# sanazkaviani/3d-latent-diffusion-model

Measured on AMD Instinct MI355X. Metric: UNet denoising steps/sec (bf16, 1x4x24x24x24 latent; whole job = sum over GPUs), higher is better.
Workload: dtype bf16

## Files before the change

### 3d-latent-diffusion-model_amd/csrc/ldm3d.hip

```cpp
#include <hip/hip_runtime.h>
#include <dlfcn.h>
#include <math.h>
#include <stdarg.h>
#include <stdio.h>
#include <stdlib.h>
#include <string.h>

#include <algorithm>
#include <atomic>
#include <map>
#include <memory>
#include <string>
#include <type_traits>
#include <vector>

#include "../../include/ldm3d.h"
#include "attention.h"
#include "conv_igemm.h"
#include "conv_halo.h"
#include "conv_cube.h"
#ifdef LDM_EXPERIMENTS
#include "conv_halo_pp.h"
#include "conv_halo_rw.h"
#endif
#include "conv_thin.h"
#include "gemm_light.h"
#include "gemm_light_x3.h"
#include "conv_block.h"
#include "conv_wgrad.h"
#include "conv_wgrad_w16.h"
#include "conv_wgrad_kw3.h"
#include "norm_elem.h"
#include "window.h"
#include "metrics.h"
#include "fin_gn.h"
#include "f32_path.h"
#include "f32_train.h"

#ifndef CONV_STAGES
#define CONV_STAGES 4
#endif

static thread_local char g_err[1024] = "";
static int fail(int code, const char* fmt, ...) {
    va_list ap; va_start(ap, fmt); vsnprintf(g_err, sizeof g_err, fmt, ap); va_end(ap);
    return code;
}
#define HIP_TRY(x) do { hipError_t e_ = (x); if (e_ != hipSuccess) \
    return fail(LDM_ERR_HIP, "%s failed: %s (%s:%d)", #x, hipGetErrorString(e_), __FILE__, __LINE__); } while (0)
#define LDM_TRY(x) do { int r_ = (x); if (r_ != 0) return r_; } while (0)


#ifdef LDM_EXPERIMENTS
// ... 68 lines not shown
struct Ref { int base = BASE_NULL; size_t off = 0; };
static inline Ref ws_ref(size_t off) { Ref r; r.base = BASE_WS; r.off = off; return r; }
static inline Ref w_ref(size_t off) { Ref r; r.base = BASE_W; r.off = off; return r; }
static inline Ref io_ref(int i) { Ref r; r.base = BASE_IO0 + i; r.off = 0; return r; }
static inline Ref w32_ref(size_t off) { Ref r; r.base = BASE_W32; r.off = 2 * off; return r; }

struct Act {
    size_t off = 0; int C = 0; int N = 0, D = 0, H = 0, W = 0; bool valid = false;
    size_t stats_off = 0; bool has_stats = false;
    int stats_nrb = 0;
    int esz = 2;
    bool hl = false;
    size_t cs_off = 0; int cs_rows = 0;
    size_t bytes() const { return (size_t)N * D * H * W * C * esz; }
    long rows() const { return (long)N * D * H * W; }
};

enum OpKind { OP_PACK, OP_CONV, OP_FINALIZE, OP_GN_STATS, OP_GN_FINALIZE, OP_GN_PREP, OP_GN_APPLY, OP_ATTN, OP_SINUSOID,
              OP_GEMV, OP_VAE_HEADS, OP_GN_FUSED,
              OP_WT , OP_WT_BATCH, OP_WGRAD, OP_EXPORT , OP_EXPORT_BATCH, OP_COLSUM, OP_GNB, OP_ATTN_BWD, OP_ADD, OP_SUMPOOL, OP_LIN_DX, OP_LIN_DW, OP_VAE_HEADS_BWD,
              OP_GEMM_LIGHT,
              OP_COLSUM_BATCH,
              OP_IM2COL,
              OP_PACK32, OP_CONV32, OP_FIN32, OP_GN_STATS32, OP_GN_APPLY32, OP_ATTN32, OP_GEMV32,
              OP_TAP,
              OP_BUCKET, OP_BUCKET_JOIN,
              OP_UPS_SPLIT32,
              OP_CONV_THIN,
              OP_FIN_GN,
              OP_GEMM_LIGHT32,
              OP_CONV_BLOCK,
              OP_TEMB_ROW };

struct ConvCfg { int wgm, wgn, bk, splitk; int halo = 0, mtps = 0, qps = 0; int slab_lg = 0; int cube = 0; int th = 0, big = 0; };

struct ConvRec {
    Ref xa, xb, w; int ca, cb;
    Ref x1a, x1b, w1; int c1a, c1b;
    int N, Din, Hin, Win, Dout, Hout, Wout;
    int k, stride, pad, M;
    int couts, cout_pad, cout_real;
    int nchunk0, nchunk1, mtiles, ntiles;
    bool ups, exact;
    bool phase;
    bool x3;
    bool ep32_ndhwc, ep32_ncdhw;
    Ref bias, bias2, temb, residual; int temb_stride;
    Ref out; int f32_out;
    Ref partial, stats;
    int stats_nrb, stats_rows;
    Ref gamma, beta, gn_out; int gn_groups, gn_silu, gn_lg; float gn_eps;
};

struct GnRec {
    Ref xa, xb; int ca, cb, N, DHW;
    Ref gamma, beta; int groups; float eps; bool silu;
    Ref stats_a, stats_b; int nrb_a, nrb_b;
    Ref partial; int nslab, rows_per_slab;
    Ref ab, mr;
    Ref out; bool out_hl;
    int rows_per_block, chunks;
    Ref dy, gsum, dgamma_n, dbeta_n;
    Ref cs; bool leaves_colsums;
    Ref acc_a, acc_b, dxa, dxb;
    int dgamma_flat, dbeta_flat;
    bool fp32;
    int count, out_stride; bool over_n;
// ... 278 lines not shown
        const ConvW* w = nullptr;
        int k = 3, stride = 1, pad = 1, ups = 0;
        int Do = 0, Ho = 0, Wo = 0;
        Act g1a, g1b; const ConvW* w1 = nullptr;
        Ref temb; int temb_stride = 0;
        Act residual;
        bool f32_out = false; Ref out_ref; int cout_real = 0;
        bool want_stats = true;
        Ref w_over; bool no_bias = false; int exact = 0;
        int temb_row = -1;
        int f32_tag = 0;
    };
    struct Tape {
        int kind = 0;
        ConvArgs c; Act out; bool leaf_input = false;
        const GnW* g = nullptr; Act xa, xb; size_t ab_off = 0, mr_off = 0; int groups = 0; bool silu = false;
        Act qkv, o; size_t lse_off = 0; int head_ch = 64;
    };
    std::vector<Tape> tape;

    static bool halo_enabled() { return ldm_knob("LDM_CONV_HALO", 1) != 0; }
    static int tall_mode() { return ldm_xknob("LDM_HALO_TALL", 2); }
    static bool light_enabled() { return ldm_knob("LDM_GEMM_LIGHT", 1) != 0; }
    static bool two_wg_enabled() { return ldm_knob("LDM_IGEMM_2WG", 1) != 0; }
    static bool phase_enabled() { return ldm_knob("LDM_CONV_PHASE", 1) != 0; }
    static bool halo_skip_enabled() { static const int v = ldm_knob("LDM_HALO_SKIP", 1); return v != 0; }
    static bool halo_skip_split_enabled() { static const int v = ldm_knob("LDM_HALO_SKIP_SPLIT", 1); return v != 0; }
    static bool cube_enabled() { return ldm_knob("LDM_CONV_CUBE", 1) != 0; }
    static bool cube_ok(int D, int H, int W, int cin0, int c1a, int c1b, int cout_pad) {
        return cube_enabled() && D >= 1 && H >= 1 && W >= 1 && D <= CUBE_EDGE && H <= CUBE_EDGE && W <= CUBE_EDGE && cin0 % 64 == 0 && cin0 >= 128 &&
               c1a % 64 == 0 && c1b % 64 == 0 && cout_pad % 16 == 0;
    }
    static ConvCfg cube_cfg(int cin0) { ConvCfg c{2, 2, 64, cin0 / 64}; c.cube = 1; return c; }
    static ConvCfg choose_cfg(long M, int cout_pad, int steps0, int bk, int halo_n = 0, long halo_dhw = 0, bool halo_only = false, int steps1 = 0) {
        ConvCfg best{2, 2, bk, 1}; double best_t = 1e30;
        const int steps = steps0 + steps1;
        const int rb = bk * 2;
        static const int splits[] = {1, 2, 3, 4, 6, 8, 9, 12, 16, 18, 24, 27, 32, 48, 64};
        for (int wgn = 1; wgn <= 4 && !halo_only; wgn *= 2) {
            const int bn = 64 * wgn, bm = 64 * (4 / wgn);
            if (cout_pad % bn) continue;
            const long tiles = ((M + bm - 1) / bm) * (cout_pad / bn);
            const double c_mfma = (double)bm * bn * bk * 2.0 / 4096.0;
            const double c_load = (double)(bm + bn) * rb / 28.0;
            const double c_step = std::max(c_mfma, c_load) + 60.0;
            for (int sk : splits) {
                if (sk > 1 && steps / sk < 6) break;
                const long nwg = tiles * sk;
                const int sps = (steps + sk - 1) / sk;
                const double rounds = ceil((double)nwg / 256.0);
                double t = rounds * (sps * c_step + 2500.0);
                if (sk > 1) t += 6000.0 + (double)M * cout_pad * 4.0 * sk * 2.0 / 2500.0;
                if (t < best_t) { best_t = t; best = ConvCfg{4 / wgn, wgn, bk, sk}; }
            }
        }
        if (halo_n > 0 && bk == 64 && cout_pad % 128 == 0 && halo_enabled()) {
            const int mtps = (int)((halo_dhw + 125) / 126), Q = steps0 / 3;
            const long tiles = (long)halo_n * mtps * (cout_pad / 128);
            const double c_mfma = 128.0 * 128.0 * 64.0 * 2.0 / 4096.0;
            const double c_load = (128.0 / 3.0 + 128.0) * 128.0 / 28.0;
            const double c_step = std::max(c_mfma, c_load) + 30.0;
            for (int sk : splits) {
                if (sk > 1 && Q / sk < 3) break;
                const int qps = (Q + sk - 1) / sk, skr = (Q + qps - 1) / qps;
                const long nwg = tiles * skr;
                const double rounds = ceil((double)nwg / 256.0);
// ... 252 lines not shown
                return Act();
            }
        }
        const bool phase = a.ups == 1 && !a.exact && a.k == 3 && a.stride == 1 && a.pad == 1 && !train && !a.xb.valid && !a.w1 &&
                           a.w_over.base == BASE_NULL && w.wp_off != 0 && phase_enabled() &&
                           a.Do == 2 * a.xa.D && a.Ho == 2 * a.xa.H && a.Wo == 2 * a.xa.W;
        if (gemm_light_ok(a.k, a.stride, a.ups, cin0, !a.w1, !a.f32_out && a.temb.base == BASE_NULL) && light_enabled() &&
            a.xa.D == a.Do && a.xa.H == a.Ho && a.xa.W == a.Wo && M * (long)cin0 * 2 < (1L << 31))
            return emit_light(OP_GEMM_LIGHT, a, M, a.w_over.base != BASE_NULL ? a.w_over : w_ref(w.w_off), gemm_light_big(M, w.cout_pad), a.want_stats);
        if (conv_block_enabled() && a.k == 3 && a.stride == 1 && a.pad == 1 && a.ups == 0 && !a.exact && !a.xb.valid && !a.w1 && !a.f32_out &&
            w.cout_pad == 64 && rup(w.cout, 32) == 64 && cin0 <= conv_block_max_cin() &&
            a.xa.D == a.Do && a.xa.H == a.Ho && a.xa.W == a.Wo) {
            const int TH = conv_block_th();
            const int td = (a.Do + BLK_TD - 1) / BLK_TD, th = (a.Ho + TH - 1) / TH, tw = (a.Wo + BLK_TW - 1) / BLK_TW;
            static const long min_blocks = ldm_knob("LDM_CONV_BLOCK_MIN", 512L);
            if ((long)N * td * th * tw >= min_blocks) return emit_conv_block(a, M, TH, td * th * tw);
        }
        if (conv_block128_enabled() && a.k == 3 && a.stride == 1 && a.pad == 1 && a.ups == 0 && !a.exact && !a.xb.valid && !a.w1 && !a.f32_out &&
            w.cout_pad == 128 && rup(w.cout, 32) == 128 && cin0 <= conv_block128_max_cin() && a.xa.D == a.Do && a.xa.H == a.Ho && a.xa.W == a.Wo) {
            const int td = (a.Do + BLK_TD - 1) / BLK_TD, th = (a.Ho + 7) / 8, tw = (a.Wo + BLK_TW - 1) / BLK_TW;
            static const long min_blocks = ldm_knob("LDM_CONV_BLOCK128_MIN", 192L);
            static const long max_blocks = ldm_xknob("LDM_CONV_BLOCK128_MAX", 0L);
            const long tiles128 = (long)N * td * th * tw;
            if (tiles128 >= min_blocks && tiles128 <= (max_blocks > 0 ? max_blocks : (long)device_cus())) return emit_conv_block(a, M, 8, td * th * tw);
        }
        const int taps = phase ? 8 : a.k * a.k * a.k;
        const bool halo_ok = a.k == 3 && a.stride == 1 && a.pad == 1 && a.ups == 0 && !a.exact && !a.xb.valid && (!a.w1 || (halo_skip_enabled() && bk == 64)) &&
                             a.xa.D == a.Do && a.xa.H == a.Ho && a.xa.W == a.Wo;
        int nchunk0 = cin0 / bk, nchunk1 = cin1 / bk;
        int steps0 = taps * nchunk0, steps1 = nchunk1;
        ConvCfg cc = choose_cfg(M, w.cout_pad, steps0, bk, halo_ok ? N : 0, (long)a.Do * a.Ho * a.Wo, false, steps1);
        if (halo_ok && bk == 64 && !hp && !train && !phase && cube_ok(a.Do, a.Ho, a.Wo, cin0, a.w1 ? a.g1a.C : 0, (a.w1 && a.g1b.valid) ? a.g1b.C : 0, w.cout_pad))
            cc = cube_cfg(cin0);
        const int bm = 64 * cc.wgm, bn = 64 * cc.wgn;
        const int couts = a.f32_out ? 0 : rup(w.cout, 32);
        const int mtiles_pp = (int)(((long)a.xa.D * a.xa.H * a.xa.W + bm - 1) / bm);
        if (!cc.halo && cc.bk == 64 && cc.wgm <= 2 && cc.splitk == 1 && two_wg_enabled() && steps0 + steps1 <= 64 &&
            (phase ? (long)N * 8 * mtiles_pp : (M + bm - 1) / bm) * (w.cout_pad / bn) >= 512) {
            cc.bk = 32; nchunk0 = cin0 / 32; nchunk1 = cin1 / 32; steps0 = taps * nchunk0; steps1 = nchunk1;
        }
        Act out;
        if (!a.f32_out) {
            out = new_act(N, a.Do, a.Ho, a.Wo, couts);
            if (a.want_stats) {
                const long dhwo = (long)a.Do * a.Ho * a.Wo;
                if (cc.splitk > 1) {
                    out.stats_off = pool.alloc((size_t)((M + 31) / 32) * couts * 2 * 4); out.has_stats = true; out.stats_nrb = 0;
                } else if (cc.halo) {
                    out.stats_off = pool.alloc((size_t)N * cc.mtps * couts * 2 * 4); out.has_stats = true; out.stats_nrb = cc.mtps;
                } else if (phase) {
                    out.stats_off = pool.alloc((size_t)N * 8 * mtiles_pp * couts * 2 * 4); out.has_stats = true; out.stats_nrb = 8 * mtiles_pp;
                } else if (N == 1 || dhwo % bm == 0) {
                    out.stats_off = pool.alloc((size_t)((M + bm - 1) / bm) * couts * 2 * 4); out.has_stats = true;
                    out.stats_nrb = (int)(N == 1 ? (M + bm - 1) / bm : dhwo / bm);
                }
            }
        }
        Op op{}; op.kind = OP_CONV; op.cc = cc;
        ConvRec& c = op.cv; c = conv_rec(a, phase ? 2 : a.k, a.stride, a.pad, M, a.cout_real ? a.cout_real : w.cout);
        conv_epilogue(c, a, out); conv_sources(c, a);
        c.w = a.w_over.base != BASE_NULL ? a.w_over : w_ref(phase ? w.wp_off : w.w_off);
        if (a.w1) {
            c.x1a = ws_ref(a.g1a.off); c.c1a = a.g1a.C; c.w1 = w_ref(a.w1->w_off); c.bias2 = w_ref(a.w1->b_off);
            if (a.g1b.valid) { c.x1b = ws_ref(a.g1b.off); c.c1b = a.g1b.C; }
        }
        c.stats = out.has_stats ? ws_ref(out.stats_off) : Ref();
        c.phase = phase; c.ups = !phase && (a.ups & 1); c.exact = !phase && (a.exact & 1);
        c.nchunk0 = nchunk0; c.nchunk1 = nchunk1;
        c.mtiles = cc.halo ? N * cc.mtps : phase ? N * 8 * mtiles_pp : (int)((M + bm - 1) / bm);
        if (M >= (1L << 31)) { err = "conv " + tag + ": M too large"; return Act(); }
        if (cc.splitk > 1) { partial_bytes = std::max(partial_bytes, (size_t)cc.splitk * M * w.cout_pad * 4); partial_fixups.push_back(plan->ops.size()); }
        plan->ops.push_back(op);
        if (cc.splitk > 1) { Op f = op; f.kind = OP_FINALIZE; partial_fixups.push_back(plan->ops.size()); plan->ops.push_back(f); }
        record_conv(a, out);
        return out;
    }

    static bool fin_gn_enabled() { static const int v = ldm_knob("LDM_FIN_GN", 1); return v != 0; }
    std::map<size_t, Act> prenorm;
    bool fuse_fin_gn(Act& raw, bool keep_raw, const GnW& g, int groups, float eps, bool silu, Act* y) {
// ... 1089 lines not shown
#define ABL_CASE(A) if ((p.dbg & 508) == A) { \
            HIP_TRY(hipFuncSetAttribute(reinterpret_cast<const void*>(&conv3_halo_kernel<6, A>), hipFuncAttributeMaxDynamicSharedMemorySize, LDS)); \
            hipLaunchKernelGGL((conv3_halo_kernel<6, A>), dim3(p.mtiles * p.ntiles * p.splitk), dim3(512), LDS, s, p); return 0; }
        if ((p.dbg & 508) == 384) {
            constexpr int LDSX = LDS + 64;
            if (p.dbg & 2048) {
                HIP_TRY(hipFuncSetAttribute(reinterpret_cast<const void*>(&conv3_halo_kernel<6, 385>), hipFuncAttributeMaxDynamicSharedMemorySize, LDSX));
                hipLaunchKernelGGL((conv3_halo_kernel<6, 385>), dim3(p.mtiles * p.ntiles * p.splitk), dim3(512), LDSX, s, p); return 0;
            }
            HIP_TRY(hipFuncSetAttribute(reinterpret_cast<const void*>(&conv3_halo_kernel<6, 384>), hipFuncAttributeMaxDynamicSharedMemorySize, LDSX));
            hipLaunchKernelGGL((conv3_halo_kernel<6, 384>), dim3(p.mtiles * p.ntiles * p.splitk), dim3(512), LDSX, s, p); return 0;
        }
        ABL_CASE(4) ABL_CASE(8) ABL_CASE(16) ABL_CASE(12) ABL_CASE(20) ABL_CASE(24) ABL_CASE(32) ABL_CASE(40) ABL_CASE(84) ABL_CASE(68) ABL_CASE(64) ABL_CASE(128) ABL_CASE(256)
#undef ABL_CASE
    }
    if (loop) hipLaunchKernelGGL((conv3_halo_kernel<6, 0, false, true>), dim3(grid), dim3(512), LDS, s, p);
    else if (mi) hipLaunchKernelGGL((conv3_halo_kernel<6, 0, false, false, true>), dim3(grid), dim3(512), LDS, s, p);
    else hipLaunchKernelGGL((conv3_halo_kernel<6>), dim3(grid), dim3(512), LDS, s, p);
    return 0;
}

static int launch_conv_cube(const ConvParams& p, hipStream_t s) {
    if (p.c0a % 64 || p.x0b || p.x3_n || p.splitk != p.c0a / 64 || p.splitk < 2 || p.CoutPad % 16 || p.Dout > CUBE_EDGE || p.Hout > CUBE_EDGE ||
        p.Wout > CUBE_EDGE || p.c1a % 64 || p.c1b % 64 || !p.partial)
        return fail(LDM_ERR_BAD_ARG, "conv3_cube_kernel: unsupported conv (cin %d, splitk %d, %dx%dx%d)", p.c0a, p.splitk, p.Dout, p.Hout, p.Wout);
    static bool attr_tab[32] = {}; bool& attr_set = attr_flag(attr_tab);
    if (!attr_set) {
        HIP_TRY(hipFuncSetAttribute(reinterpret_cast<const void*>(&conv3_cube_kernel), hipFuncAttributeMaxDynamicSharedMemorySize, CUBE_LDS));
        attr_set = true;
    }
    hipLaunchKernelGGL(conv3_cube_kernel, dim3(p.splitk, p.CoutPad / 16, p.N), dim3(256), CUBE_LDS, s, p);
    return 0;
}
static int launch_conv_impl(const ConvParams& p, const ConvCfg& cc, hipStream_t s) {
    if (cc.cube) return launch_conv_cube(p, s);
    if (cc.halo) return launch_conv_halo(p, s, cc.halo == 2);
#define CASE(M_, N_, K_) if (cc.wgm == M_ && cc.wgn == N_ && cc.bk == K_) return launch_conv_t<M_, N_, K_>(p, s);
    CASE(2, 2, 64) CASE(4, 1, 64) CASE(1, 4, 64) CASE(2, 2, 32) CASE(4, 1, 32) CASE(1, 4, 32)
#undef CASE
    return fail(LDM_ERR_BAD_ARG, "no conv kernel for tile config %dx%d bk %d", cc.wgm, cc.wgn, cc.bk);
}

static inline int grid_for(long total, int per_block = 256, int cap = 4096) {
    long g = (total + per_block - 1) / per_block; if (g > cap) g = cap; if (g < 1) g = 1; return (int)g;
}

static void conv32_cfg(long M, int cout_pad, int steps, bool x3, int* bn_out, int* sk_out) {
    static const int f32_bn = ldm_knob("LDM_F32_BN", 0);
    static const int f32_wgs = ldm_knob("LDM_F32_WGS", 512);
    const int mtiles = (int)((M + 127) / 128);
    int bn = (cout_pad % 128) ? 64 : 128;
    if (f32_bn == 64 || (f32_bn == 1 && (long)mtiles * (cout_pad / 128) < 256)) bn = 64;
    const long tiles = (long)mtiles * ((cout_pad + bn - 1) / bn);
    int sk = 1;
    if (tiles < f32_wgs * 3 / 4) {
        sk = (int)std::min<long>(std::max<long>(1, f32_wgs / tiles), std::max(1, steps / (x3 ? 4 : 8)));
        const int sps = (steps + sk - 1) / sk; sk = (steps + sps - 1) / sps;
    }
    *bn_out = bn; *sk_out = sk;
}
static int fin32_stats_blocks(int N, int dhwo, int couts, int* rows) {
    const int cvec = couts / 4, rows_par = std::max(1, 256 / cvec);
    int nrb = std::min((dhwo + rows_par - 1) / rows_par, std::max(1, 256 / N));
    *rows = (dhwo + nrb - 1) / nrb;
    return (dhwo + *rows - 1) / *rows;
}
static void launch_conv32(const Conv32Params& p, bool x3, int bn, hipStream_t s) {
    const dim3 grid(p.mtiles * p.ntiles * p.splitk);
// ... 199 lines not shown
template <class P> static P wgrad_params(const WgradRec& w, const Bases& bs) {
    P p{}; p.dy = (decltype(p.dy))rp(bs, w.dy); p.cdy = w.cdy; p.x = (decltype(p.x))rp(bs, w.x); p.cx = w.cx;
    p.dw = (float*)rp(bs, w.dw); p.Cout = w.Cout; p.Cin = w.Cin; p.dw_ld = w.dw_ld; p.dw_ci_off = w.dw_ci_off;
    p.N = w.N; p.Din = w.Din; p.Hin = w.Hin; p.Win = w.Win; p.Dout = w.Dout; p.Hout = w.Hout; p.Wout = w.Wout;
    p.ksize = w.ksize; p.stride = w.stride; p.pad = w.pad; p.ups = w.ups; p.M = w.M;
    p.co_tiles = (p.Cout + 127) / 128; p.ci_tiles = (p.Cin + 127) / 128; p.ksplit = w.ksplit;
    p.slab_stride = (long)w.ksize * w.ksize * w.ksize * w.rows_total * w.dw_ld;
    return p;
}

struct PlanTrace { bool on = false; std::string path; PlanTrace() { const char* e = getenv("LDM_PLAN_TRACE"); if (e && *e) { on = true; path = e; } } };
static PlanTrace g_plan_trace;
struct LaneCtx { GradSyncState* sync = nullptr; };

static int run_plan(const Plan& plan, const Bases& bs, const int* rt, hipStream_t s, size_t begin = 0, size_t end = (size_t)-1,
                    LaneCtx lanes = LaneCtx()) {
    if (end > plan.ops.size()) end = plan.ops.size();
    const char* trace_path = g_plan_trace.on ? g_plan_trace.path.c_str() : nullptr;
    std::vector<hipEvent_t> tev;
    if (trace_path) { tev.resize(end - begin + 1); for (auto& e : tev) HIP_TRY(hipEventCreate(&e)); }
    struct TraceDone {
        const Plan& plan; size_t begin, end; std::vector<hipEvent_t>& ev; hipStream_t s; const char* path;
        ~TraceDone() {
            if (ev.empty()) return;
            (void)hipEventRecord(ev.back(), s); (void)hipEventSynchronize(ev.back());
            FILE* f = fopen(path, "a");
            for (size_t oi = begin; oi < end && f; ++oi) {
                const Op& o = plan.ops[oi]; float ms = 0.f; (void)hipEventElapsedTime(&ms, ev[oi - begin], ev[oi - begin + 1]);
                fprintf(f, "%zu,%zu,%d,%.3f", plan.ops.size(), oi, (int)o.kind, ms * 1e3f);
                const ConvRec& c = o.cv;
                if (o.kind == OP_CONV || o.kind == OP_FINALIZE)
                    fprintf(f, ",M=%d k=%d s=%d ups=%d cin=%d+%d(x%d) cin1=%d couts=%d cfg=%dx%dx%d splitk=%d halo=%d mtps=%d qps=%d cube=%d", c.M, c.k, c.stride,
                            c.ups | c.exact << 1 | c.phase << 2 | c.x3 << 3 | c.ep32_ndhwc << 4 | c.ep32_ncdhw << 5, c.ca, c.cb, c.nchunk0, c.c1a + c.c1b, c.couts,
                            o.cc.wgm, o.cc.wgn, o.cc.bk, o.cc.splitk, o.cc.halo, o.cc.mtps, o.cc.qps, o.cc.cube);
                else {
                    const GnRec& g = o.gn; const WgradRec& w = o.wg;
                    int v[6] = {o.i[0], o.i[1], o.i[2], o.i[3], o.i[4], o.i[5]};
                    auto six = [&](int a, int b, int c2, int d, int e, int h) { v[0] = a; v[1] = b; v[2] = c2; v[3] = d; v[4] = e; v[5] = h; };
                    switch (o.kind) {
                        case OP_FIN_GN: six(c.gn_groups, c.gn_silu, c.gn_lg, c.c1b, c.N, c.Din); break;
                        case OP_CONV32: case OP_FIN32: six(c.ca, c.cb, c.stats_nrb, c.stats_rows, c.N, c.Din); break;
                        case OP_CONV_THIN: six(c.N, c.Din, c.Hin, c.Win, c.x3 ? c.ca / 2 * 3 : c.ca, c.cout_pad); break;
                        case OP_CONV_BLOCK: six(c.N, c.Dout, c.Hout, c.Wout, c.ca, o.cc.th); break;
                        case OP_GEMM_LIGHT: case OP_GEMM_LIGHT32: six(c.M, c.ca + c.cb, c.couts, c.cout_pad, o.cc.big, c.ca); break;
                        case OP_GN_STATS: case OP_GN_STATS32: six(g.ca, g.cb, g.DHW, g.nslab, g.rows_per_slab, g.N); break;
                        case OP_GN_FINALIZE: six(g.nslab, g.ca + g.cb, g.groups, g.DHW, g.N, 0); break;
                        case OP_GN_PREP: six(g.ca, g.cb, g.nrb_a, g.groups, g.DHW, g.N); break;
                        case OP_GN_FUSED: six(g.ca, g.cb, g.nrb_a, g.nrb_b, g.groups, g.DHW); break;
                        case OP_GN_APPLY: six(g.ca, g.cb, g.DHW, g.N, g.silu, 0); break;
                        case OP_GN_APPLY32: six(g.ca, g.cb, g.DHW, g.N, g.silu, g.nrb_a ? 1 : g.nslab); break;
                        case OP_COLSUM: six(g.N, g.nslab, g.ca, g.over_n, g.count, g.out_stride); break;
                        case OP_GNB: six(g.ca, g.cb, g.groups, g.DHW, g.N, g.silu); break;
                        case OP_WGRAD: six(w.cdy, w.cx, w.Cout, w.Cin, w.dw_ld, w.dw_ci_off); break;
                        default: break;
                    }
                    fprintf(f, ",i=%d %d %d %d %d %d", v[0], v[1], v[2], v[3], v[4], v[5]);
                }
                fprintf(f, "\n");
            }
            if (f) fclose(f);
            for (auto e : ev) (void)hipEventDestroy(e);
        }
    } trace_done{plan, begin, end, tev, s, trace_path};
    for (size_t oi = begin; oi < end; ++oi) {
        const Op& o = plan.ops[oi];
        const int* i = o.i;
        if (trace_path) HIP_TRY(hipEventRecord(tev[oi - begin], s));
// ... 1338 lines not shown
    for (auto& e : g_prof.ev) HIP_TRY(hipEventCreate(&e));
    g_prof.wgm = wgm; g_prof.wgn = wgn; g_prof.bk = bk & 0xff; g_prof.halo = (bk >> 8) & 1; g_prof.on = true;
    return 0;
}
int ldm_profile_detail(double* flops, double* ms, int max) {
    if (!flops || !ms || max < 0) return fail(LDM_ERR_BAD_ARG, "null argument");
    const int n = (int)(g_prof.used / 2);
    for (int k = 0; k < n && k < max; ++k) {
        HIP_TRY(hipEventSynchronize(g_prof.ev[2 * k + 1]));
        float t = 0.f; HIP_TRY(hipEventElapsedTime(&t, g_prof.ev[2 * k], g_prof.ev[2 * k + 1]));
        flops[k] = g_prof.flops[k]; ms[k] = t;
    }
    return n;
}
int ldm_profile_stop(double out[5]) {
    if (!out) return fail(LDM_ERR_BAD_ARG, "null out");
    g_prof.on = false;
    double ms = 0.0, fl = 0.0;
    for (size_t k = 0; k + 1 < g_prof.used + 1 && k < g_prof.used; k += 2) {
        HIP_TRY(hipEventSynchronize(g_prof.ev[k + 1]));
        float t = 0.f; HIP_TRY(hipEventElapsedTime(&t, g_prof.ev[k], g_prof.ev[k + 1]));
        ms += t; fl += g_prof.flops[k / 2];
    }
    out[0] = (double)(g_prof.used / 2); out[1] = ms; out[2] = fl; out[3] = (double)g_prof.launches_all; out[4] = g_prof.flops_all;
    for (auto e : g_prof.ev) (void)hipEventDestroy(e);
    g_prof.ev.clear(); g_prof.used = 0; g_prof.flops.clear();
    return 0;
}
int ldm_model_plan_conv_cfgs(ldm_model* m, const char* kind, int B, int D, int H, int W, int* cfgs, int max_convs) {
    if (!m || !kind) return fail(LDM_ERR_BAD_ARG, "null argument");
    std::shared_ptr<Plan> p; LDM_TRY(get_plan(m, kind, B, D, H, W, &p));
    int n = 0;
    for (const Op& o : p->ops) if (o.kind == OP_CONV) {
        if (cfgs && n < max_convs) { cfgs[4 * n] = o.cc.wgm; cfgs[4 * n + 1] = o.cc.wgn; cfgs[4 * n + 2] = o.cc.bk | ((o.cc.cube ? 5 : o.cc.halo) << 8); cfgs[4 * n + 3] = o.cc.splitk; }
        ++n;
    } else if (o.kind == OP_CONV_BLOCK) {
        if (cfgs && n < max_convs) { cfgs[4 * n] = 4; cfgs[4 * n + 1] = o.cv.couts == 128 ? 2 : 1; cfgs[4 * n + 2] = 32 | ((o.cv.couts == 128 ? 4 : 3) << 8); cfgs[4 * n + 3] = 1; }
        ++n;
    }
    return n;
}

int ldm_model_plan_launches(ldm_model* m, const char* kind, int B, int D, int H, int W) {
    if (!m || !kind) return fail(LDM_ERR_BAD_ARG, "null argument");
    std::shared_ptr<Plan> p; LDM_TRY(get_plan(m, kind, B, D, H, W, &p));
    int n = 0;
    for (const Op& o : p->ops) if (o.kind != OP_TAP) ++n;
    return n;
}

static char* g_zero_page = nullptr;
static int ensure_zero_page() {
    if (g_zero_page) return 0;
    HIP_TRY(hipMalloc((void**)&g_zero_page, 8192));
    HIP_TRY(hipMemset(g_zero_page, 0, 8192));
    HIP_TRY(hipDeviceSynchronize());
    return 0;
}

int ldm_op_conv3d_block128(const void* x, int cin, const void* w, const float* bias, const float* temb, int temb_stride, const void* residual,
                           void* out, float* stats, int N, int D, int H, int W, void* stream) {
    if (!x || !w || !out || N < 1 || D < 1 || H < 1 || W < 1 || cin < 32 || cin % 32) return fail(LDM_ERR_BAD_ARG, "bad argument");
    if ((long)N * D * H * W * cin * 2 >= (1L << 32)) return fail(LDM_ERR_BAD_ARG, "the input tensor exceeds 4 GiB (split the batch)");
    BlockParams q{}; q.x = (const bf16_t*)x; q.w = (const bf16_t*)w; q.bias = bias; q.temb = temb; q.temb_stride = temb_stride;
    q.residual = (const bf16_t*)residual; q.out = (bf16_t*)out; q.stats = stats; q.N = N; q.D = D; q.H = H; q.W = W; q.Cin = cin;
    HIP_TRY(launch_conv_block128(q, (hipStream_t)stream));
    return 0;
// ... 43 lines not shown
    const int Du = Din << ups, Hu = Hin << ups, Wu = Win << ups;
    const int pad_total = (stride == 2 && pad == 0 && ksize == 3) ? 1 : 2 * pad;
    const int Do = (Du + pad_total - ksize) / stride + 1, Ho = (Hu + pad_total - ksize) / stride + 1,
              Wo = (Wu + pad_total - ksize) / stride + 1;
    const long M = (long)N * Do * Ho * Wo;
    if (M >= (1L << 31) || M < 1) return fail(LDM_ERR_BAD_ARG, "bad output size");
    if (!stats && !wgn && !splitk && out_bf16 && !out_f32 && gemm_light_ok(ksize, stride, ups, cin0, cin1 == 0, !temb && !bias2) &&
        Builder::light_enabled() && M * (long)cin0 * 2 < (1L << 31)) {
        LightParams lp{}; lp.x = (const bf16_t*)xa; lp.w = (const bf16_t*)w; lp.bias = bias; lp.residual = (const bf16_t*)residual;
        lp.out = (bf16_t*)out_bf16; lp.stats = nullptr; lp.M = (int)M; lp.K = cin0; lp.CoutS = rup(cout, 32);
        lp.xb = (const bf16_t*)xb; lp.ca = ca;
        HIP_TRY(launch_gemm_light(lp, cout_pad, gemm_light_big(M, cout_pad), (hipStream_t)stream));
        return 0;
    }
    const int taps = ksize * ksize * ksize;
    ConvParams p{};
    p.x0a = (const bf16_t*)xa; p.x0b = (const bf16_t*)xb; p.c0a = ca; p.c0b = cb; p.w0 = (const bf16_t*)w;
    p.x1a = (const bf16_t*)x1a; p.x1b = (const bf16_t*)x1b; p.c1a = c1a; p.c1b = c1b; p.w1 = (const bf16_t*)w1;
    p.zero_page = (const bf16_t*)g_zero_page;
    p.N = N; p.Din = Din; p.Hin = Hin; p.Win = Win; p.Dout = Do; p.Hout = Ho; p.Wout = Wo;
    p.ksize = ksize; p.stride = stride; p.pad = pad; p.ups = ups; p.exact = exact; p.M = (int)M;
    p.CoutS = rup(cout, 32); p.CoutPad = cout_pad; p.CoutReal = cout;
    p.nchunk0 = cin0 / bk; p.nchunk1 = cin1 / bk; p.steps0 = taps * p.nchunk0; p.steps1 = p.nchunk1;
    const bool halo_ok = ksize == 3 && stride == 1 && pad == 1 && ups == 0 && !exact && cb == 0 && bk == 64 &&
                         (cin1 == 0 || (Builder::halo_skip_enabled() && (splitk <= 1 || Builder::halo_skip_split_enabled()))) && Builder::halo_enabled();
    ConvCfg cc = Builder::choose_cfg(M, cout_pad, p.steps0, bk, halo_ok ? N : 0, (long)Do * Ho * Wo, false, p.steps1);
    if (wgn) {
        if ((wgn != 1 && wgn != 2 && wgn != 4) || cout_pad % (64 * wgn)) return fail(LDM_ERR_BAD_ARG, "bad wgn");
        cc.wgn = wgn; cc.wgm = 4 / wgn; cc.halo = (wgn == 2 && halo_ok && cout_pad % 128 == 0) ? 1 : (wgn == 1 && halo_ok && Builder::tall_mode() != 0) ? 2 : 0;
    }
    if (splitk) cc.splitk = splitk;
    if (!wgn && !splitk && halo_ok && !out_f32 && !(ldm_xknob("LDM_CONV_DBG", 0)) && Builder::cube_ok(Do, Ho, Wo, cin0, c1a, c1b, cout_pad))
        cc = Builder::cube_cfg(cin0);
    if (cc.splitk < 1 || cc.splitk > p.steps0 + p.steps1) return fail(LDM_ERR_BAD_ARG, "bad splitk");
    if (cc.halo && !cc.cube) {
        const int Q = 9 * p.nchunk0;
        if (cc.splitk > Q) cc.splitk = Q;
        cc.qps = (Q + cc.splitk - 1) / cc.splitk; cc.splitk = (Q + cc.qps - 1) / cc.qps;
        cc.mtps = (int)(((long)Do * Ho * Wo + (cc.halo == 2 ? 253 : 125)) / (cc.halo == 2 ? 254 : 126));
    }
    p.splitk = cc.splitk; p.steps_per_split = cc.halo ? 3 * cc.qps : (p.steps0 + p.steps1 + cc.splitk - 1) / cc.splitk;
    p.halo_mtps = cc.mtps; p.q_per_split = cc.qps;
    p.mtiles = cc.halo ? N * cc.mtps : (int)((M + 64 * cc.wgm - 1) / (64 * cc.wgm)); p.ntiles = cout_pad / (64 * cc.wgn);
    p.bias = bias; p.bias2 = bias2; p.temb = temb; p.temb_stride = temb_stride; p.residual = (const bf16_t*)residual;
    p.out = out_f32 ? nullptr : (bf16_t*)out_bf16; p.out_f32 = out_f32;
    if (cc.splitk > 1) {
        const size_t need = (size_t)cc.splitk * M * cout_pad * 4;
        if (!scratch || scratch_bytes < need) return fail(LDM_ERR_WORKSPACE, "split-K scratch too small: need %zu bytes", need);
        p.partial = (float*)scratch;
    }
    if (stats) {
        const long dhwo = (long)Do * Ho * Wo; const int bm = 64 * cc.wgm;
        if (out_f32 || !stats_nrb) return fail(LDM_ERR_BAD_ARG, "statistics need the bf16 output form");
        if (cc.splitk > 1) { if (N > 1 && dhwo % 32) return fail(LDM_ERR_UNSUPPORTED, "statistics: DHW %% 32 != 0 with a batch"); *stats_nrb = (int)(N == 1 ? (M + 31) / 32 : dhwo / 32); }
        else if (cc.halo) *stats_nrb = cc.mtps;
        else { if (N > 1 && dhwo % bm) return fail(LDM_ERR_UNSUPPORTED, "statistics: tiles straddle samples"); *stats_nrb = (int)(N == 1 ? (M + bm - 1) / bm : dhwo / bm); }
        p.stats = stats;
    }
    p.dbg = (int)ldm_xknob("LDM_CONV_DBG", 0);
    if (p.dbg & 512) {
        if (cc.splitk > 1 || !scratch || scratch_bytes < (size_t)p.mtiles * p.ntiles * (64 + 4096)) return fail(LDM_ERR_BAD_ARG, "stamps need scratch and splitk 1");
        p.stamps = (unsigned long long*)scratch;
    }
    if (fg && cc.splitk > 1) p.slab_lg = fg->lg;
    LDM_TRY(launch_conv(p, cc, (hipStream_t)stream));
    if (cc.splitk > 1) {
        const FinalizeParams f = finalize_params(p);
        if (fg) {
            fg->f = f; fg->f.stats = nullptr;
            HIP_TRY(launch_fin_gn(*fg, N, wt_stores(), (hipStream_t)stream));
        } else
            launch_finalize(f, stats && wt_stores(), (hipStream_t)stream);
    } else if (fg) return fail(LDM_ERR_UNSUPPORTED, "the fused finalize + GroupNorm needs a conv that is split over K");
    HIP_TRY(hipGetLastError());
    return 0;
}

int ldm_op_conv3d(const void* xa, int ca, const void* xb, int cb, const void* w, const float* bias,
                  const void* x1a, int c1a, const void* x1b, int c1b, const void* w1, const float* bias2,
                  const float* temb, int temb_stride, const void* residual, void* out_bf16, float* out_f32,
                  int N, int Din, int Hin, int Win, int ksize, int stride, int pad, int ups,
                  int cout, int cout_pad, int wgn, int splitk, void* scratch, size_t scratch_bytes, void* stream) {
    return op_conv3d_impl(xa, ca, xb, cb, w, bias, x1a, c1a, x1b, c1b, w1, bias2, temb, temb_stride, residual, out_bf16, out_f32, N, Din, Hin, Win,
                          ksize, stride, pad, ups, cout, cout_pad, wgn, splitk, scratch, scratch_bytes, stream, nullptr, nullptr);
}

size_t ldm_op_conv3d_gn_scratch_bytes(int N, int D, int H, int W, int cout_pad, int splitk) {
// ... 1009 lines not shown
```

Measured before the change: 508.1.

## Add plane-per-workgroup 3x3x3 conv kernel for 12^3 feature maps

Adds a new conv kernel that gives each workgroup one output depth plane and a 16-channel output slice. It stages the three input planes plus all 27 tap weights in LDS through buffer-load-to-LDS with dedicated loader waves, and double-buffers the stages. It covers volumes up to 12^3 that are too large for the cube kernel, and fuses the skip-connection 1x1 conv, bias, temb, residual and per-plane GroupNorm stats. The aim is to replace split-K or halo paths and their finalize passes at mid resolution, at the cost of one-workgroup-per-CU occupancy and a large LDS footprint.

```diff
diff --git a/3d-latent-diffusion-model_amd/csrc/conv_plane.h b/3d-latent-diffusion-model_amd/csrc/conv_plane.h
--- /dev/null
+++ b/3d-latent-diffusion-model_amd/csrc/conv_plane.h
@@ -0,0 +1,230 @@
+#pragma once
+#include <type_traits>
+#include "conv_cube.h"
+
+constexpr int PLANE_EDGE = 12;
+constexpr int PLANE_ROWS = 576;
+constexpr int PLANE_TILES = 10;
+constexpr int PLANE_IMG = PLANE_ROWS * 64;
+constexpr int PLANE_STAGE = PLANE_IMG + 27 * 1024;
+constexpr int PLANE_SROWS = 192;
+constexpr int PLANE_SUNIT = 8 * PLANE_SROWS * 16;
+constexpr int PLANE_SWOFF = 2 * PLANE_SUNIT;
+constexpr int PLANE_RED = 16384;
+constexpr int PLANE_LDS = 2 * PLANE_STAGE;
+static_assert(PLANE_LDS <= 160 * 1024, "LDS budget");
+static_assert(PLANE_ROWS % 64 == 0 && PLANE_SROWS % 64 == 0, "whole LDS-DMA copies; chunk strides a multiple of 16 rows");
+static_assert(PLANE_TILES * 16 >= PLANE_EDGE * (PLANE_EDGE + 1), "tiles cover the domain");
+static_assert(PLANE_TILES * 16 - 1 + 2 * (PLANE_EDGE + 1) * (PLANE_EDGE + 1) + 2 * (PLANE_EDGE + 1) + 2 < PLANE_ROWS, "largest row read");
+static_assert(PLANE_TILES * 16 <= PLANE_SROWS && PLANE_SWOFF + 2 * 2048 <= PLANE_STAGE, "skip stage fits a stage buffer");
+static_assert(PLANE_TILES * 1024 <= PLANE_RED && PLANE_RED + 256 <= PLANE_LDS, "end-of-kernel areas");
+
+__global__ __launch_bounds__(512, 1) __attribute__((amdgpu_waves_per_eu(2, 2))) void conv3_plane_kernel(const ConvParams p) {
+#if defined(__HIP_DEVICE_COMPILE__)
+    extern __shared__ __attribute__((aligned(16))) char smem[];
+    typedef __attribute__((address_space(3))) void* lds_ptr_t;
+    constexpr unsigned OOB = 0x80000000u;
+    const int tid = threadIdx.x, lane = tid & 63;
+    const int wave8 = __builtin_amdgcn_readfirstlane(tid >> 6);
+    const bool loader = wave8 >= 4;
+    const int wave = wave8 & 3;
+    const int n0 = blockIdx.x * 16, d = blockIdx.y, smp = blockIdx.z;
+    if (n0 >= p.CoutS) return;
+    const int D = p.Dout, H = p.Hout, W = p.Wout, DHW = D * H * W, RP = W + 1, PP = (H + 1) * RP, dom = H * RP;
+    const unsigned cin2 = (unsigned)p.c0a * 2u;
+    const int nst0 = p.c0a >> 5, units = p.steps1, nst = nst0 + ((units + 1) >> 1);
+
+    const bf16_t* xs = p.x0a + (size_t)smp * DHW * p.c0a;
+    __amdgpu_buffer_rsrc_t rs_x = __builtin_amdgcn_make_buffer_rsrc((void*)xs, 0, (int)((unsigned)DHW * cin2), 0x00020000);
+    __amdgpu_buffer_rsrc_t rs_w = __builtin_amdgcn_make_buffer_rsrc((void*)p.w0, 0, (int)(27u * (unsigned)p.CoutPad * cin2), 0x00020000);
+    unsigned vo[PLANE_ROWS / 64];
+#pragma unroll
+    for (int i = 0; i < PLANE_ROWS / 64; ++i) {
+        const int r = (wave + 4 * i) * 16 + (lane >> 2);
+        const int pl = r / PP, rem = r - pl * PP, hp = rem / RP, wp = rem - hp * RP, dd = d - 1 + pl;
+        const bool real = pl <= 2 && dd >= 0 && dd < D && hp >= 1 && wp >= 1;
+        vo[i] = real ? (unsigned)((dd * H + hp - 1) * W + wp - 1) * cin2 + (unsigned)(lane & 3) * 16u : OOB;
+    }
+    const unsigned wv = (unsigned)(wave * p.CoutPad + n0 + (lane >> 2)) * cin2 + (unsigned)((lane & 3) ^ ((lane >> 3) & 2)) * 16u;
+    const unsigned wstep = 4u * (unsigned)p.CoutPad * cin2;
+    auto issue_main = [&](const int s, const int b) {
+        char* buf = smem + b * PLANE_STAGE;
+        const unsigned so = (unsigned)s * 64u;
+#pragma unroll
+        for (int i = 0; i < 7; ++i) {
+            const int tap = wave + 4 * i;
+            if (tap < 27) __builtin_amdgcn_raw_ptr_buffer_load_lds(rs_w, (lds_ptr_t)(buf + PLANE_IMG + tap * 1024), 16, wv + (unsigned)i * wstep + so, 0, 0, 0);
+        }
+#pragma unroll
+        for (int i = 0; i < PLANE_ROWS / 64; ++i)
+            __builtin_amdgcn_raw_ptr_buffer_load_lds(rs_x, (lds_ptr_t)(buf + (wave + 4 * i) * 1024), 16, vo[i] + so, 0, 0, 0);
+    };
+    unsigned s_vox[PLANE_SROWS / 64];
+#pragma unroll
+    for (int g = 0; g < PLANE_SROWS / 64; ++g) {
+        const int q = g * 64 + lane;
+        s_vox[g] = OOB;
+        if (q < dom) {
+            const int h = q / RP, w = q - h * RP;
+            if (w < W) s_vox[g] = (unsigned)((d * H + h) * W + w);
+        }
+    }
+    const int nca = p.c1a / 64;
+    const unsigned w1row2 = (unsigned)(p.c1a + p.c1b) * 2u;
+    auto issue_skip = [&](const int j, const int b) {
+        char* buf = smem + b * PLANE_STAGE;
+#pragma unroll
+        for (int ul = 0; ul < 2; ++ul) {
+            const int u = 2 * j + ul;
+            if (u >= units) break;
+            const bool a = u < nca;
+            const bf16_t* src = (a ? p.x1a : p.x1b) + (size_t)smp * DHW * (a ? p.c1a : p.c1b);
+            const unsigned row2 = (unsigned)(a ? p.c1a : p.c1b) * 2u, jc = (unsigned)(a ? u : u - nca) * 128u;
+            __amdgpu_buffer_rsrc_t rs_s = __builtin_amdgcn_make_buffer_rsrc((void*)src, 0, (int)((unsigned)DHW * row2), 0x00020000);
+#pragma unroll
+            for (int i = 0; i < 2 * (PLANE_SROWS / 64); ++i) {
+                const int ch = wave + 4 * (i & 1), g = i >> 1;
+                const unsigned v = s_vox[g] != OOB ? s_vox[g] * row2 + jc + (unsigned)ch * 16u : OOB;
+                __builtin_amdgcn_raw_ptr_buffer_load_lds(rs_s, (lds_ptr_t)(buf + ul * PLANE_SUNIT + ch * (PLANE_SROWS * 16) + g * 1024), 16, v, 0, 0, 0);
+            }
+            if ((wave >> 1) == ul) {
+                const int hf = wave & 1;
+                __amdgpu_buffer_rsrc_t rs_1w = __builtin_amdgcn_make_buffer_rsrc((void*)p.w1, 0, (int)((unsigned)p.CoutPad * w1row2), 0x00020000);
+                const unsigned v = (unsigned)(n0 + (lane & 15)) * w1row2 + (unsigned)u * 128u + (unsigned)(hf * 4 + (lane >> 4)) * 16u;
+                __builtin_amdgcn_raw_ptr_buffer_load_lds(rs_1w, (lds_ptr_t)(buf + PLANE_SWOFF + ul * 2048 + hf * 1024), 16, v, 0, 0, 0);
+            }
+        }
+    };
+    auto issue = [&](const int s) { if (s < nst0) issue_main(s, s & 1); else issue_skip(s - nst0, s & 1); };
+    if (loader) issue(0);
+
+    const int mh = wave & 1, kh = wave >> 1;
+    const int fr = lane & 15, kq = lane >> 4;
+    int abase[9][5];
+#pragma unroll
+    for (int t = 0; t < 5; ++t) {
+        const int q = (mh * 5 + t) * 16 + fr;
+        const int a0 = kq * 16 + (q < dom ? q : 0) * 64;
+#pragma unroll
+        for (int j = 0; j < 9; ++j) abase[j][t] = a0 + ((j / 3) * PP + (j % 3) * RP) * 64;
+    }
+    const int wbase = PLANE_IMG + fr * 64 + (kq ^ ((fr >> 1) & 2)) * 16;
+    f32x4 acc[5];
+#pragma unroll
+    for (int t = 0; t < 5; ++t) acc[t] = (f32x4){0.f, 0.f, 0.f, 0.f};
+
+    auto taps = [&](auto boc, auto t0c, auto t1c) {
+        constexpr int BO = decltype(boc)::value, T0 = decltype(t0c)::value, T1 = decltype(t1c)::value;
+        bf16x8 wf[2], af[2][5];
+        wf[0] = *reinterpret_cast<const bf16x8*>(smem + wbase + (BO + T0 * 1024));
+#pragma unroll
+        for (int t = 0; t < 5; ++t) af[0][t] = *reinterpret_cast<const bf16x8*>(smem + abase[T0 / 3][t] + (BO + (T0 % 3) * 64));
+#pragma unroll
+        for (int k = T0; k < T1; ++k) {
+            const int cur = (k - T0) & 1, nxt = cur ^ 1;
+            if (k + 1 < T1) {
+                const int k1 = k + 1;
+                wf[nxt] = *reinterpret_cast<const bf16x8*>(smem + wbase + (BO + k1 * 1024));
+#pragma unroll
+                for (int t = 0; t < 5; ++t) af[nxt][t] = *reinterpret_cast<const bf16x8*>(smem + abase[k1 / 3][t] + (BO + (k1 % 3) * 64));
+            }
+#pragma unroll
+            for (int t = 0; t < 5; ++t) acc[t] = __builtin_amdgcn_mfma_f32_16x16x32_bf16(wf[cur], af[cur][t], acc[t], 0, 0, 0);
+#pragma unroll
+            for (int t = 0; t < 5; ++t) { __builtin_amdgcn_sched_group_barrier(0x008, 1, 0); __builtin_amdgcn_sched_group_barrier(0x100, 1, 0); }
+            __builtin_amdgcn_sched_group_barrier(0x100, 1, 0);
+            __builtin_amdgcn_sched_barrier(0);
+        }
+    };
+
+    for (int s = 0; s < nst; ++s) {
+        if (loader) asm volatile("s_waitcnt vmcnt(0)" ::: "memory");
+        cube_barrier();
+        if (loader) {
+            if (s + 1 < nst) issue(s + 1);
+            continue;
+        }
+        const int bo = (s & 1) * PLANE_STAGE;
+        if (s < nst0) {
+            typedef std::integral_constant<int, 0> B0; typedef std::integral_constant<int, PLANE_STAGE> B1;
+            typedef std::integral_constant<int, 14> T14; typedef std::integral_constant<int, 27> T27;
+            if (kh == 0) { if (s & 1) taps(B1{}, B0{}, T14{}); else taps(B0{}, B0{}, T14{}); }
+            else { if (s & 1) taps(B1{}, T14{}, T27{}); else taps(B0{}, T14{}, T27{}); }
+        } else {
+            const int nu = units - 2 * (s - nst0) < 2 ? units - 2 * (s - nst0) : 2;
+            for (int ul = 0; ul < nu; ++ul) {
+                const int ch = kh * 4 + kq;
+                const bf16x8 sw = *reinterpret_cast<const bf16x8*>(smem + bo + PLANE_SWOFF + ul * 2048 + ch * 256 + fr * 16);
+#pragma unroll
+                for (int t = 0; t < 5; ++t) {
+                    const bf16x8 sa = *reinterpret_cast<const bf16x8*>(smem + bo + ul * PLANE_SUNIT + ch * (PLANE_SROWS * 16) + ((mh * 5 + t) * 16 + fr) * 16);
+                    acc[t] = __builtin_amdgcn_mfma_f32_16x16x32_bf16(sw, sa, acc[t], 0, 0, 0);
+                }
+            }
+        }
+    }
+
+    const int c = n0 + 4 * kq;
+    float4 eb = make_float4(0.f, 0.f, 0.f, 0.f), et = eb;
+    if (kh == 0 && !loader) {
+        if (p.bias) eb = *reinterpret_cast<const float4*>(p.bias + c);
+        if (p.bias2) { const float4 b2 = *reinterpret_cast<const float4*>(p.bias2 + c); eb.x += b2.x; eb.y += b2.y; eb.z += b2.z; eb.w += b2.w; }
+        if (p.temb) et = *reinterpret_cast<const float4*>(p.temb + (size_t)smp * p.temb_stride + c);
+    }
+    cube_barrier();
+    float4* xch = reinterpret_cast<float4*>(smem);
+    if (kh == 1 && !loader) {
+#pragma unroll
+        for (int t = 0; t < 5; ++t) xch[(mh * 5 + t) * 64 + lane] = make_float4(acc[t][0], acc[t][1], acc[t][2], acc[t][3]);
+    }
+    cube_barrier();
+    float ssum[4] = {0.f, 0.f, 0.f, 0.f}, ssq[4] = {0.f, 0.f, 0.f, 0.f};
+    if (kh == 0 && !loader) {
+#pragma unroll
+        for (int t = 0; t < 5; ++t) {
+            const int q = (mh * 5 + t) * 16 + fr;
+            if (q >= dom) continue;
+            const int h = q / RP, w = q - h * RP;
+            if (w >= W) continue;
+            const float4 o = xch[(mh * 5 + t) * 64 + lane];
+            float v[4] = {acc[t][0] + o.x, acc[t][1] + o.y, acc[t][2] + o.z, acc[t][3] + o.w};
+            if (p.bias || p.bias2) { v[0] += eb.x; v[1] += eb.y; v[2] += eb.z; v[3] += eb.w; }
+            if (p.temb) { v[0] += et.x; v[1] += et.y; v[2] += et.z; v[3] += et.w; }
+            const size_t m = (size_t)smp * DHW + (size_t)((d * H + h) * W + w);
+            if (p.residual) {
+                const u32x2 rv = *reinterpret_cast<const u32x2*>(p.residual + m * p.CoutS + c);
+                v[0] += __uint_as_float(rv[0] << 16); v[1] += __uint_as_float(rv[0] & 0xffff0000u);
+                v[2] += __uint_as_float(rv[1] << 16); v[3] += __uint_as_float(rv[1] & 0xffff0000u);
+            }
+            u32x2 ov;
+            ov[0] = pack2bf(v[0], v[1]); ov[1] = pack2bf(v[2], v[3]);
+#pragma unroll
+            for (int i = 0; i < 2; ++i) {
+                const float lo = __uint_as_float(ov[i] << 16), hi = __uint_as_float(ov[i] & 0xffff0000u);
+                ssum[2 * i] += lo; ssq[2 * i] += lo * lo; ssum[2 * i + 1] += hi; ssq[2 * i + 1] += hi * hi;
+            }
+            *reinterpret_cast<u32x2*>(p.out + m * p.CoutS + c) = ov;
+        }
+    }
+    if (p.stats) {
+        float* red = reinterpret_cast<float*>(smem + PLANE_RED);
+        if (kh == 0 && !loader) {
+#define PLANE_ROW_ADD(X, CTRL) X += __int_as_float(__builtin_amdgcn_update_dpp(0, __float_as_int(X), CTRL, 0xf, 0xf, true))
+#pragma unroll
+            for (int r = 0; r < 4; ++r) {
+                PLANE_ROW_ADD(ssum[r], 0x128); PLANE_ROW_ADD(ssum[r], 0x124); PLANE_ROW_ADD(ssum[r], 0x122); PLANE_ROW_ADD(ssum[r], 0x121);
+                PLANE_ROW_ADD(ssq[r], 0x128); PLANE_ROW_ADD(ssq[r], 0x124); PLANE_ROW_ADD(ssq[r], 0x122); PLANE_ROW_ADD(ssq[r], 0x121);
+            }
+#undef PLANE_ROW_ADD
+            if (fr == 0) {
+#pragma unroll
+                for (int r = 0; r < 4; ++r) { red[(mh * 16 + 4 * kq + r) * 2] = ssum[r]; red[(mh * 16 + 4 * kq + r) * 2 + 1] = ssq[r]; }
+            }
+        }
+        cube_barrier();
+        if (tid < 16)
+            *reinterpret_cast<float2*>(p.stats + (((size_t)smp * D + d) * p.CoutS + n0 + tid) * 2) =
+                make_float2(red[tid * 2] + red[(16 + tid) * 2], red[tid * 2 + 1] + red[(16 + tid) * 2 + 1]);
+    }
+#endif
+}
diff --git a/3d-latent-diffusion-model_amd/csrc/ldm3d.hip b/3d-latent-diffusion-model_amd/csrc/ldm3d.hip
--- a/3d-latent-diffusion-model_amd/csrc/ldm3d.hip
+++ b/3d-latent-diffusion-model_amd/csrc/ldm3d.hip
@@ -19,6 +19,7 @@
 #include "conv_igemm.h"
 #include "conv_halo.h"
 #include "conv_cube.h"
+#include "conv_plane.h"
 #ifdef LDM_EXPERIMENTS
 #include "conv_halo_pp.h"
 #include "conv_halo_rw.h"
@@ -153,7 +154,7 @@
               OP_CONV_BLOCK,
               OP_TEMB_ROW };
 
-struct ConvCfg { int wgm, wgn, bk, splitk; int halo = 0, mtps = 0, qps = 0; int slab_lg = 0; int cube = 0; int th = 0, big = 0; };
+struct ConvCfg { int wgm, wgn, bk, splitk; int halo = 0, mtps = 0, qps = 0; int slab_lg = 0; int cube = 0; int th = 0, big = 0; int plane = 0; };
 
 struct ConvRec {
     Ref xa, xb, w; int ca, cb;
@@ -498,6 +499,14 @@
                c1a % 64 == 0 && c1b % 64 == 0 && cout_pad % 16 == 0;
     }
     static ConvCfg cube_cfg(int cin0) { ConvCfg c{2, 2, 64, cin0 / 64}; c.cube = 1; return c; }
+    static bool plane_enabled() { return ldm_knob("LDM_CONV_PLANE", 1) != 0; }
+    static int plane_max_cin() { return (int)ldm_knob("LDM_CONV_PLANE_MAX_CIN", 256); }
+    static bool plane_ok(int D, int H, int W, int cin0, int c1a, int c1b, int cout_pad) {
+        return plane_enabled() && D >= 1 && H >= 1 && W >= 1 && D <= PLANE_EDGE && H <= PLANE_EDGE && W <= PLANE_EDGE &&
+               (D > CUBE_EDGE || H > CUBE_EDGE || W > CUBE_EDGE) && cin0 % 64 == 0 && cin0 >= 128 && cin0 <= plane_max_cin() &&
+               c1a % 64 == 0 && c1b % 64 == 0 && cout_pad % 16 == 0;
+    }
+    static ConvCfg plane_cfg() { ConvCfg c{2, 2, 64, 1}; c.plane = 1; return c; }
     static ConvCfg choose_cfg(long M, int cout_pad, int steps0, int bk, int halo_n = 0, long halo_dhw = 0, bool halo_only = false, int steps1 = 0) {
         ConvCfg best{2, 2, bk, 1}; double best_t = 1e30;
         const int steps = steps0 + steps1;
@@ -816,10 +825,13 @@
         ConvCfg cc = choose_cfg(M, w.cout_pad, steps0, bk, halo_ok ? N : 0, (long)a.Do * a.Ho * a.Wo, false, steps1);
         if (halo_ok && bk == 64 && !hp && !train && !phase && cube_ok(a.Do, a.Ho, a.Wo, cin0, a.w1 ? a.g1a.C : 0, (a.w1 && a.g1b.valid) ? a.g1b.C : 0, w.cout_pad))
             cc = cube_cfg(cin0);
+        else if (halo_ok && bk == 64 && !hp && !train && !phase && !a.f32_out &&
+                 plane_ok(a.Do, a.Ho, a.Wo, cin0, a.w1 ? a.g1a.C : 0, (a.w1 && a.g1b.valid) ? a.g1b.C : 0, w.cout_pad))
+            cc = plane_cfg();
         const int bm = 64 * cc.wgm, bn = 64 * cc.wgn;
         const int couts = a.f32_out ? 0 : rup(w.cout, 32);
         const int mtiles_pp = (int)(((long)a.xa.D * a.xa.H * a.xa.W + bm - 1) / bm);
-        if (!cc.halo && cc.bk == 64 && cc.wgm <= 2 && cc.splitk == 1 && two_wg_enabled() && steps0 + steps1 <= 64 &&
+        if (!cc.halo && !cc.plane && cc.bk == 64 && cc.wgm <= 2 && cc.splitk == 1 && two_wg_enabled() && steps0 + steps1 <= 64 &&
             (phase ? (long)N * 8 * mtiles_pp : (M + bm - 1) / bm) * (w.cout_pad / bn) >= 512) {
             cc.bk = 32; nchunk0 = cin0 / 32; nchunk1 = cin1 / 32; steps0 = taps * nchunk0; steps1 = nchunk1;
         }
@@ -830,6 +842,8 @@
                 const long dhwo = (long)a.Do * a.Ho * a.Wo;
                 if (cc.splitk > 1) {
                     out.stats_off = pool.alloc((size_t)((M + 31) / 32) * couts * 2 * 4); out.has_stats = true; out.stats_nrb = 0;
+                } else if (cc.plane) {
+                    out.stats_off = pool.alloc((size_t)N * a.Do * couts * 2 * 4); out.has_stats = true; out.stats_nrb = a.Do;
                 } else if (cc.halo) {
                     out.stats_off = pool.alloc((size_t)N * cc.mtps * couts * 2 * 4); out.has_stats = true; out.stats_nrb = cc.mtps;
                 } else if (phase) {
@@ -1985,8 +1999,22 @@
     hipLaunchKernelGGL(conv3_cube_kernel, dim3(p.splitk, p.CoutPad / 16, p.N), dim3(256), CUBE_LDS, s, p);
     return 0;
 }
+static int launch_conv_plane(const ConvParams& p, hipStream_t s) {
+    if (p.c0a % 64 || p.c0a < 128 || p.x0b || p.x3_n || p.splitk != 1 || p.CoutPad % 16 || p.CoutS % 32 || p.Dout > PLANE_EDGE || p.Hout > PLANE_EDGE ||
+        p.Wout > PLANE_EDGE || p.Dout < 1 || p.Hout < 1 || p.Wout < 1 || p.ksize != 3 || p.stride != 1 || p.pad != 1 || p.ups || p.phase_mode ||
+        p.c1a % 64 || p.c1b % 64 || p.steps1 != (p.c1a + p.c1b) / 64 || !p.out || p.out_f32 || p.out32 || p.raw_partial)
+        return fail(LDM_ERR_BAD_ARG, "conv3_plane_kernel: unsupported conv (cin %d, splitk %d, %dx%dx%d)", p.c0a, p.splitk, p.Dout, p.Hout, p.Wout);
+    static bool attr_tab[32] = {}; bool& attr_set = attr_flag(attr_tab);
+    if (!attr_set) {
+        HIP_TRY(hipFuncSetAttribute(reinterpret_cast<const void*>(&conv3_plane_kernel), hipFuncAttributeMaxDynamicSharedMemorySize, PLANE_LDS));
+        attr_set = true;
+    }
+    hipLaunchKernelGGL(conv3_plane_kernel, dim3(p.CoutPad / 16, p.Dout, p.N), dim3(512), PLANE_LDS, s, p);
+    return 0;
+}
 static int launch_conv_impl(const ConvParams& p, const ConvCfg& cc, hipStream_t s) {
     if (cc.cube) return launch_conv_cube(p, s);
+    if (cc.plane) return launch_conv_plane(p, s);
     if (cc.halo) return launch_conv_halo(p, s, cc.halo == 2);
 #define CASE(M_, N_, K_) if (cc.wgm == M_ && cc.wgn == N_ && cc.bk == K_) return launch_conv_t<M_, N_, K_>(p, s);
     CASE(2, 2, 64) CASE(4, 1, 64) CASE(1, 4, 64) CASE(2, 2, 32) CASE(4, 1, 32) CASE(1, 4, 32)
@@ -2252,7 +2280,7 @@
                 if (o.kind == OP_CONV || o.kind == OP_FINALIZE)
                     fprintf(f, ",M=%d k=%d s=%d ups=%d cin=%d+%d(x%d) cin1=%d couts=%d cfg=%dx%dx%d splitk=%d halo=%d mtps=%d qps=%d cube=%d", c.M, c.k, c.stride,
                             c.ups | c.exact << 1 | c.phase << 2 | c.x3 << 3 | c.ep32_ndhwc << 4 | c.ep32_ncdhw << 5, c.ca, c.cb, c.nchunk0, c.c1a + c.c1b, c.couts,
-                            o.cc.wgm, o.cc.wgn, o.cc.bk, o.cc.splitk, o.cc.halo, o.cc.mtps, o.cc.qps, o.cc.cube);
+                            o.cc.wgm, o.cc.wgn, o.cc.bk, o.cc.splitk, o.cc.plane ? 6 : o.cc.halo, o.cc.mtps, o.cc.qps, o.cc.cube);
                 else {
                     const GnRec& g = o.gn; const WgradRec& w = o.wg;
                     int v[6] = {o.i[0], o.i[1], o.i[2], o.i[3], o.i[4], o.i[5]};
@@ -3657,7 +3685,7 @@
     std::shared_ptr<Plan> p; LDM_TRY(get_plan(m, kind, B, D, H, W, &p));
     int n = 0;
     for (const Op& o : p->ops) if (o.kind == OP_CONV) {
-        if (cfgs && n < max_convs) { cfgs[4 * n] = o.cc.wgm; cfgs[4 * n + 1] = o.cc.wgn; cfgs[4 * n + 2] = o.cc.bk | ((o.cc.cube ? 5 : o.cc.halo) << 8); cfgs[4 * n + 3] = o.cc.splitk; }
+        if (cfgs && n < max_convs) { cfgs[4 * n] = o.cc.wgm; cfgs[4 * n + 1] = o.cc.wgn; cfgs[4 * n + 2] = o.cc.bk | ((o.cc.cube ? 5 : o.cc.plane ? 6 : o.cc.halo) << 8); cfgs[4 * n + 3] = o.cc.splitk; }
         ++n;
     } else if (o.kind == OP_CONV_BLOCK) {
         if (cfgs && n < max_convs) { cfgs[4 * n] = 4; cfgs[4 * n + 1] = o.cv.couts == 128 ? 2 : 1; cfgs[4 * n + 2] = 32 | ((o.cv.couts == 128 ? 4 : 3) << 8); cfgs[4 * n + 3] = 1; }
@@ -3767,6 +3795,8 @@
     if (splitk) cc.splitk = splitk;
     if (!wgn && !splitk && halo_ok && !out_f32 && !(ldm_xknob("LDM_CONV_DBG", 0)) && Builder::cube_ok(Do, Ho, Wo, cin0, c1a, c1b, cout_pad))
         cc = Builder::cube_cfg(cin0);
+    else if (!wgn && !splitk && halo_ok && out_bf16 && !out_f32 && !fg && !(ldm_xknob("LDM_CONV_DBG", 0)) && Builder::plane_ok(Do, Ho, Wo, cin0, c1a, c1b, cout_pad))
+        cc = Builder::plane_cfg();
     if (cc.splitk < 1 || cc.splitk > p.steps0 + p.steps1) return fail(LDM_ERR_BAD_ARG, "bad splitk");
     if (cc.halo && !cc.cube) {
         const int Q = 9 * p.nchunk0;
@@ -3788,6 +3818,7 @@
         const long dhwo = (long)Do * Ho * Wo; const int bm = 64 * cc.wgm;
         if (out_f32 || !stats_nrb) return fail(LDM_ERR_BAD_ARG, "statistics need the bf16 output form");
         if (cc.splitk > 1) { if (N > 1 && dhwo % 32) return fail(LDM_ERR_UNSUPPORTED, "statistics: DHW %% 32 != 0 with a batch"); *stats_nrb = (int)(N == 1 ? (M + 31) / 32 : dhwo / 32); }
+        else if (cc.plane) *stats_nrb = Do;
         else if (cc.halo) *stats_nrb = cc.mtps;
         else { if (N > 1 && dhwo % bm) return fail(LDM_ERR_UNSUPPORTED, "statistics: tiles straddle samples"); *stats_nrb = (int)(N == 1 ? (M + bm - 1) / bm : dhwo / bm); }
         p.stats = stats;
```

Result: faster. 517.3, median of 6 (+1.8%).
